# heliaxdev/ark-plonk

Hardware: AMD Instinct MI355X
Metric: proofs/sec at 2^20 constraints (BLS12-381, KZG10); MSM G1-adds/s (higher is better)
Workload: dtype u32 limbs (256/384-bit Montgomery integers)

## Files before the change

### ark_plonk_amd/csrc/fieldu.cuh

```cuda
#pragma once
#include "field_common.cuh"

template <class P>
struct Fu {
    static constexpr int NL = P::NL;
    static constexpr int SAT = P::SAT_WORDS;
    static constexpr uint32_t M = (1u << 29) - 1u;
    uint32_t v[NL];

    ZK_HD static Fu zero() {
        Fu r;
#pragma unroll
        for (int i = 0; i < NL; ++i) r.v[i] = 0;
        return r;
    }
    ZK_HD static Fu one() {
        Fu r;
#pragma unroll
        for (int i = 0; i < NL; ++i) r.v[i] = P::ONE(i);
        return r;
    }
    ZK_HD bool limbs_zero() const {
        uint32_t o = 0;
#pragma unroll
// ... 119 lines not shown
            t += (uint64_t)m[k] * P::MOD(0);
            carry = t >> 29;
        }
#pragma unroll
        for (int k = NL; k < 2 * NL - 1; ++k) {
            uint64_t a0 = 0, a1 = 0, am = 0;
#pragma unroll
            for (int i = k - NL + 1; i < NL; ++i) {
                if (i & 1) a1 += (uint64_t)a.v[i] * b.v[k - i];
                else a0 += (uint64_t)a.v[i] * b.v[k - i];
                am += (uint64_t)m[i] * P::MOD(k - i);
            }
            uint64_t t = a0 + a1 + am + carry;
            r.v[k - NL] = (uint32_t)t & M;
            carry = t >> 29;
        }
        r.v[NL - 1] = (uint32_t)carry;
        return r;
    }
    ZK_HD static uint64_t fence64(uint64_t t) {
#if defined(__HIP_DEVICE_COMPILE__)
        asm("" : "+v"(t));
#endif
        return t;
    }
    ZK_HD static Fu mul_fenced(const Fu& a, const Fu& b) {
        uint32_t m[NL];
        Fu r;
        uint64_t carry = 0;
#pragma unroll
        for (int k = 0; k < NL; ++k) {
            uint64_t t = fence64(carry + (uint64_t)a.v[0] * b.v[k]);
#pragma unroll
            for (int i = 1; i <= k; ++i) t += (uint64_t)a.v[i] * b.v[k - i];
#pragma unroll
            for (int i = 0; i < k; ++i) t += (uint64_t)m[i] * P::MOD(k - i);
            m[k] = ((uint32_t)t * P::PINV) & M;
            t += (uint64_t)m[k] * P::MOD(0);
            carry = t >> 29;
        }
#pragma unroll
        for (int k = NL; k < 2 * NL - 1; ++k) {
            uint64_t t = fence64(carry + (uint64_t)a.v[k - NL + 1] * b.v[NL - 1]);
#pragma unroll
            for (int i = k - NL + 2; i < NL; ++i) t += (uint64_t)a.v[i] * b.v[k - i];
#pragma unroll
            for (int i = k - NL + 1; i < NL; ++i) t += (uint64_t)m[i] * P::MOD(k - i);
            r.v[k - NL] = (uint32_t)t & M;
            carry = t >> 29;
        }
        r.v[NL - 1] = (uint32_t)carry;
        return r;
    }
    ZK_HD static Fu sqr(const Fu& a) {
        uint32_t m[NL], a2[NL];
        Fu r;
#pragma unroll
        for (int i = 0; i < NL; ++i) a2[i] = a.v[i] << 1;
        uint64_t carry = 0;
#pragma unroll
        for (int k = 0; k < NL; ++k) {
            uint64_t aa = 0, am = 0;
#pragma unroll
            for (int i = 0; 2 * i < k; ++i) aa += (uint64_t)a2[i] * a.v[k - i];
            if ((k & 1) == 0) aa += (uint64_t)a.v[k / 2] * a.v[k / 2];
#pragma unroll
            for (int i = 0; i < k; ++i) am += (uint64_t)m[i] * P::MOD(k - i);
            uint64_t t = aa + am + carry;
            m[k] = ((uint32_t)t * P::PINV) & M;
            t += (uint64_t)m[k] * P::MOD(0);
            carry = t >> 29;
        }
#pragma unroll
        for (int k = NL; k < 2 * NL - 1; ++k) {
            uint64_t aa = 0, am = 0;
#pragma unroll
            for (int i = k - NL + 1; 2 * i < k; ++i) aa += (uint64_t)a2[i] * a.v[k - i];
            if ((k & 1) == 0) aa += (uint64_t)a.v[k / 2] * a.v[k / 2];
#pragma unroll
            for (int i = k - NL + 1; i < NL; ++i) am += (uint64_t)m[i] * P::MOD(k - i);
            uint64_t t = aa + am + carry;
            r.v[k - NL] = (uint32_t)t & M;
            carry = t >> 29;
        }
        r.v[NL - 1] = (uint32_t)carry;
        return r;
    }

    ZK_HD bool is_zero_mod_reduced() const {
        if (v[0] != 0 && v[0] != P::MOD(0)) return false;
        uint32_t dz = 0, dp = 0;
#pragma unroll
        for (int i = 0; i < NL; ++i) {
            dz |= v[i];
            dp |= v[i] ^ P::MOD(i);
        }
        return dz == 0 || dp == 0;
    }
    ZK_HD bool is_zero_mod() const { return mul(*this, one()).is_zero_mod_reduced(); }

    ZK_HD static Fu canonical_lt2p(const Fu& a) {
        Fu d;
#pragma unroll
        for (int i = 0; i < NL; ++i) d.v[i] = a.v[i] - P::MOD(i);
        normalize(d);
        const bool neg = ((int32_t)d.v[NL - 1]) < 0;
// ... 46 lines not shown
```

### ark_plonk_amd/csrc/ntt.hip

```cpp
#include "ctx.h"
#include "domain.cuh"

#include "ntt_pass.cuh"

namespace {

template <class Fr>
struct PowBits {
    Fr p[32];
};
template <class Fr>
__global__ void gen_pow_table(void* out, uint64_t n, PowBits<Fr> pb, Fr mul, int mode, uint32_t log_m, uint32_t log_mprev, Fr to_rp) {
    uint64_t i = (uint64_t)blockIdx.x * blockDim.x + threadIdx.x;
    if (i >= n) return;
    uint64_t e = i;
    if (mode == 1) {
        uint64_t col = i & ((1ull << log_m) - 1);
        uint64_t k = i >> log_m;
        e = (col * k) & ((1ull << log_mprev) - 1);
    }
    Fr r = mul;
    for (int b = 0; b < 32; ++b) {
        if ((e >> b) & 1ull) r = Fr::mul(r, pb.p[b]);
    }
// ... 108 lines not shown
    if (hipMalloc(&p, cnt * TW_INNER_U4 * 16) != hipSuccess) {
        (void)hipFree(packed);
        return ZK_ERR_OOM;
    }
    Fr w = domain_root<C>((uint32_t)s);
    if (inverse) w = Fr::inverse(w);
    int rc = launch_pow_table<C>(c, packed, cnt, w, Fr::one(), 0, 0, 0);
    if (!rc) {
        const int T = 256;
        hipLaunchKernelGGL(split_table<typename C::FrU>, dim3((unsigned)((cnt + T - 1) / T)), dim3(T), 0, c->stream, packed, p, cnt);
        if (hipGetLastError() != hipSuccess || hipStreamSynchronize(c->stream) != hipSuccess) rc = ZK_ERR_HIP;
    }
    (void)hipFree(packed);
    if (rc) {
        (void)hipFree(p);
        return rc;
    }
    c->inner_tw[key] = p;
    *out = p;
    return ZK_OK;
}

template <class C>
int get_plan(zk_ctx* c, uint32_t log_n, bool inverse, NttPlan** out) {
    typedef typename C::Fr Fr;
    const int forced = forced_passes(c, log_n);
    uint64_t key = ((uint64_t)C::ID << 40) | ((uint64_t)forced << 36) | ((uint64_t)(inverse ? 1 : 0) << 32) | log_n;
    auto it = c->plans.find(key);
    if (it != c->plans.end()) {
        *out = it->second;
        return ZK_OK;
    }
    int n_pass, s[4];
    if (!decompose(log_n, forced, n_pass, s)) return ZK_ERR_UNSUPPORTED;
    NttPlan* pl = new NttPlan();
    pl->curve = C::ID;
    pl->log_n = log_n;
    pl->inverse = inverse;
    pl->n_pass = n_pass;
    for (int i = 0; i < 4; ++i) pl->s[i] = s[i];
    uint32_t log_mprev = log_n;
    for (int p = 0; p < pl->n_pass; ++p) {
        if (log_n >= 3) {
            int rc = get_inner_tw<C>(c, pl->s[p], inverse, &pl->tw_inner[p]);
            if (rc) { delete pl; return rc; }
        }
        if (p + 1 < pl->n_pass) {
            uint32_t log_m = log_mprev - (uint32_t)pl->s[p];
            uint64_t cnt = 1ull << log_mprev;
            hipError_t e = hipMalloc(&pl->tw_pass[p], cnt * sizeof(Fr));
            if (e != hipSuccess) { delete pl; return ZK_ERR_OOM; }
            Fr w = domain_root<C>(log_mprev);
            if (inverse) w = Fr::inverse(w);
            int rc = launch_pow_table<C>(c, pl->tw_pass[p], cnt, w, Fr::one(), 1, log_m, log_mprev);
            if (rc) { delete pl; return rc; }
            log_mprev = log_m;
        }
    }
    c->plans[key] = pl;
    *out = pl;
    return ZK_OK;
}

template <class C>
int ensure_coset(zk_ctx* c, bool inv, uint64_t len, void** out) {
    typedef typename C::Fr Fr;
    DevBuf& buf = inv ? c->coset_inv_pow[C::ID] : c->coset_pow[C::ID];
    size_t& have = inv ? c->coset_inv_len[C::ID] : c->coset_len[C::ID];
    if (have < len) {
        ZK_HIP_TRY(hipStreamSynchronize(c->stream));
        uint64_t want = 1;
        while (want < len) want <<= 1;
        int rc = buf.ensure(want * sizeof(Fr));
        if (rc) return rc;
        Fr g = coset_gen<C>();
        if (inv) g = Fr::inverse(g);
        rc = launch_pow_table<C>(c, buf.p, want, g, Fr::one(), 0, 0, 0);
        if (rc) return rc;
        have = want;
    }
    *out = buf.p;
    return ZK_OK;
}

typedef int (*NttPassLauncher)(int final_pass, const NttPassArgs* a, hipStream_t st);
extern "C" NttPassLauncher zk_ntt_pass_launcher(int curve, int s);

template <class C>
int dispatch_pass(zk_ctx* c, int s, bool final_pass, const NttPassArgs& a) {
    if (s < 3 || s > 9) return ZK_ERR_UNSUPPORTED;
    NttPassLauncher fn = zk_ntt_pass_launcher(C::ID, s);
    if (!fn) return ZK_ERR_UNSUPPORTED;
    hipError_t e = (hipError_t)fn(final_pass ? 1 : 0, &a, c->stream);
    ZK_HIP_TRY(e);
    return ZK_OK;
}

template <class C>
int ntt_run(zk_ctx* c, int kind, uint32_t log_n, uint32_t n_polys, const void* const* d_ins, const size_t* in_lens, void* const* d_outs) {
    typedef typename C::Fr Fr;
    if (!domain_log_ok<C>(log_n)) return ZK_ERR_DOMAIN_TOO_LARGE;
    if (n_polys == 0 || n_polys > 16) return ZK_ERR_BAD_ARG;
    const uint64_t N = 1ull << log_n;
    size_t in_len = 0;
    bool all_quarter = true;
    for (uint32_t i = 0; i < n_polys; ++i) {
        if (in_lens[i] > N) return ZK_ERR_BAD_ARG;
// ... 32 lines not shown
        rc = ensure_coset<C>(c, true, N, &post);
        if (rc) return rc;
    }
    NttPlan* pl = nullptr;
    rc = get_plan<C>(c, log_n, inverse, &pl);
    if (rc) return rc;
    if (pl->n_pass > 4) return ZK_ERR_UNSUPPORTED;
    void* work = nullptr;
    if (pl->n_pass > 1) {
        rc = c->ntt_work.ensure((size_t)n_polys * N * sizeof(Fr));
        if (rc) return rc;
        work = c->ntt_work.p;
    }
    uint32_t log_mprev = log_n;
    NttPassArgs a;
    ProfScope ps(c, "ntt_pass");
    for (int p = 0; p < pl->n_pass; ++p) {
        const int s = pl->s[p];
        const bool last = (p + 1 == pl->n_pass);
        memset(&a, 0, sizeof a);
        a.log_n = log_n;
        a.in = (p == 0) ? d_in : work;
        a.out = last ? d_out : work;
        a.in_len = (p == 0) ? in_lens[0] : N;
        if (n_polys > 1) {
            a.n_batch = n_polys;
            for (uint32_t i = 0; i < n_polys; ++i) {
                void* wk = (char*)work + (size_t)i * N * sizeof(Fr);
                a.ins[i] = (p == 0) ? d_ins[i] : wk;
                a.outs[i] = last ? d_outs[i] : wk;
                a.in_lens[i] = (p == 0) ? in_lens[i] : N;
            }
        }
        a.tw_inner = pl->tw_inner[p];
        a.pre_mul = (p == 0) ? pre : nullptr;
        const uint32_t LC = 9u - (uint32_t)s;
        if (!last) {
            uint32_t log_m = log_mprev - (uint32_t)s;
            uint32_t logc = LC < log_m ? LC : log_m;
            a.logc = logc;
            a.log_m = log_m;
            a.log_mprev = log_mprev;
            a.tw_pass = pl->tw_pass[p];
            a.n_tiles = (uint32_t)(N >> ((uint32_t)s + logc));
            a.quarter = (p == 0 && s >= 3 && all_quarter) ? 1u : 0u;
            log_mprev = log_m;
        } else {
            uint32_t s1 = (pl->n_pass > 1) ? (uint32_t)pl->s[0] : 0;
            uint32_t logc = LC < s1 ? LC : s1;
            a.logc = logc;
            a.s1 = s1;
            a.s2 = pl->n_pass == 4 ? (uint32_t)pl->s[1] : 0u;
            a.post_mul = post;
            const Fr sc = to_rprime(inverse ? n_inv : Fr::one());
            for (int i = 0; i < 8; ++i) a.scale[i] = sc.v[i];
            a.n_tiles = (uint32_t)(N >> ((uint32_t)s + logc));
        }
        rc = dispatch_pass<C>(c, s, last, a);
        if (rc) return rc;
        if (c->profiling) c->prof["ntt_passes"].launches += 1;
    }
    return ZK_OK;
}

}

int ntt_run_dev(zk_ctx* c, int curve, int kind, uint32_t log_n, const void* d_in, size_t in_len, void* d_out) {
    return ntt_run_batch_dev(c, curve, kind, log_n, 1, &d_in, &in_len, &d_out);
}

int ntt_run_batch_dev(zk_ctx* c, int curve, int kind, uint32_t log_n, uint32_t n_polys, const void* const* d_ins, const size_t* in_lens,
                      void* const* d_outs) {
    if (kind < 0 || kind > 3) return ZK_ERR_BAD_ARG;
    for (uint32_t base = 0; base < n_polys; base += 16) {
        const uint32_t cnt = n_polys - base < 16 ? n_polys - base : 16;
        const int rc = zk_on_curve(curve, ZK_ERR_BAD_ARG, [&](auto cv) {
            return ntt_run<decltype(cv)>(c, kind, log_n, cnt, d_ins + base, in_lens + base, d_outs + base);
        });
        if (rc) return rc;
    }
    return ZK_OK;
}

int ntt_prepare(zk_ctx* c, int curve, uint32_t log_n) {
    NttPlan* pl;
    if (log_n < 3) return ZK_OK;
    for (int inv = 0; inv < 2; ++inv) {
        const int rc = zk_on_curve(curve, ZK_ERR_BAD_ARG, [&](auto cv) {
            typedef decltype(cv) Cv;
            if (!domain_log_ok<Cv>(log_n)) return ZK_ERR_DOMAIN_TOO_LARGE;
            return get_plan<Cv>(c, log_n, inv != 0, &pl);
        });
        if (rc) return rc;
    }
    return ZK_OK;
}

void ntt_ctx_free(zk_ctx* c) {
    for (auto& kv : c->plans) delete kv.second;
    c->plans.clear();
    for (auto& kv : c->inner_tw) (void)hipFree(kv.second);
    c->inner_tw.clear();
    c->ntt_work.release();
    for (int i = 0; i < 2; ++i) {
        c->coset_pow[i].release();
        c->coset_inv_pow[i].release();
    }
}
// ... 34 lines not shown
```

### ark_plonk_amd/csrc/ntt_pass.cuh

```cuda
#pragma once
#include <hip/hip_runtime.h>
#include "curve_params.h"
#include "field.cuh"
#include "fieldu.cuh"

typedef __attribute__((address_space(3))) volatile uint32_t lds_u32;

struct NttPassArgs {
    const void* in;
    void* out;
    const void* tw_inner;
    const void* tw_pass;
    const void* pre_mul;
    const void* post_mul;
    uint32_t scale[8];
    uint64_t in_len;
    uint32_t log_n;
    uint32_t logc;
    uint32_t log_m;
    uint32_t log_mprev;
    uint32_t s1;
    uint32_t s2;
    uint32_t n_tiles;
    uint32_t quarter;
    uint32_t n_batch;
    const void* ins[16];
    void* outs[16];
    uint64_t in_lens[16];
};

__host__ __device__ inline uint32_t bitrev32(uint32_t x, int bits) {
#if defined(__HIP_DEVICE_COMPILE__)
    return bits ? __brev(x) >> (32 - bits) : 0u;
#else
    uint32_t r = 0;
    for (int i = 0; i < bits; ++i) { r = (r << 1) | (x & 1); x >>= 1; }
    return r;
#endif
}

template <class F>
ZK_D F ld_u(const void* base, uint64_t idx) {
    const uint4* q = reinterpret_cast<const uint4*>(base) + 2 * idx;
    uint4 a = q[0], b = q[1];
    uint32_t w[8] = {a.x, a.y, a.z, a.w, b.x, b.y, b.z, b.w};
    return F::split_words(w);
}
template <class F>
ZK_D void st_u(void* base, uint64_t idx, const F& x) {
    uint32_t w[8];
    F::canonical_lt2p(x).pack_words(w);
    uint4* q = reinterpret_cast<uint4*>(base) + 2 * idx;
    q[0] = make_uint4(w[0], w[1], w[2], w[3]);
    q[1] = make_uint4(w[4], w[5], w[6], w[7]);
}

template <class F>
ZK_D void st_u_raw(void* base, uint64_t idx, const F& x) {
    uint32_t w[8];
    x.pack_words(w);
    uint4* q = reinterpret_cast<uint4*>(base) + 2 * idx;
    q[0] = make_uint4(w[0], w[1], w[2], w[3]);
    q[1] = make_uint4(w[4], w[5], w[6], w[7]);
}

constexpr int TW_INNER_U4 = 3;
template <class F>
ZK_D F ld_limbs(const void* base, uint64_t idx) {
    static_assert(F::NL <= 4 * TW_INNER_U4, "inner twiddle entry too small");
    const uint4* q = reinterpret_cast<const uint4*>(base) + TW_INNER_U4 * idx;
    F r;
#pragma unroll
    for (int i = 0; i < TW_INNER_U4; ++i) {
        if (4 * i >= F::NL) break;
        const uint4 a = q[i];
        if (4 * i + 0 < F::NL) r.v[4 * i + 0] = a.x;
        if (4 * i + 1 < F::NL) r.v[4 * i + 1] = a.y;
// ... 19 lines not shown
ZK_D uint32_t window_pos(uint32_t v, uint32_t e) {
    return ((v >> B0) << (B0 + 3)) | (e << B0) | (v & ((1u << B0) - 1u));
}

template <class F>
ZK_D void wave_exchange(F (&x)[8], lds_u32* sc, const uint32_t (&widx)[8], const uint32_t (&ridx)[8]) {
#pragma unroll
    for (int l = 0; l < F::NL; ++l) {
#pragma unroll
        for (int e = 0; e < 8; ++e) sc[widx[e]] = x[e].v[l];
        __builtin_amdgcn_wave_barrier();
#pragma unroll
        for (int e = 0; e < 8; ++e) x[e].v[l] = sc[ridx[e]];
        __builtin_amdgcn_wave_barrier();
    }
}

template <class F, int S, int B0, int LB_LO, int LB_HI>
ZK_D void dit_window(F (&x)[8], uint32_t v, const void* tw, bool quarter) {
    const uint32_t vlow = v & ((1u << B0) - 1u);
#pragma unroll
    for (int lb = LB_LO; lb < LB_HI; ++lb) {
        const int t = B0 + lb;
        if (ntt_sweep_at(t)) {
#pragma unroll
            for (int e = 0; e < 8; ++e) F::sweep(x[e]);
        }
#pragma unroll
        for (int e = 0; e < 8; ++e) {
            if (e & (1 << lb)) continue;
            const int eo = e | (1 << lb);
            if constexpr (B0 == 0 && LB_LO == 0) {
                if (lb < 2 && quarter) {
                    x[eo] = x[e];
                    continue;
                }
                if (lb == 0) {
                    const F b = x[eo];
                    x[eo] = F::sub_raw3(x[e], b);
                    x[e] = F::add_raw(x[e], b);
                    continue;
                }
                if ((e & ((1 << lb) - 1)) == 0) {
                    F b = x[eo];
                    F::sweep(b);
                    x[eo] = lb == 1 ? F::sub_raw8(x[e], b) : F::sub_raw16(x[e], b);
                    x[e] = F::add_raw(x[e], b);
                    continue;
                }
            }
            const uint32_t plow = ((uint32_t)(e & ((1 << lb) - 1)) << B0) | vlow;
            const uint32_t j = plow << (S - 1 - t);
            F w = ld_limbs<F>(tw, j);
            F m = F::mul_fenced(x[eo], w);
            x[eo] = F::sub_raw3(x[e], m);
            x[e] = F::add_raw(x[e], m);
        }
    }
}

template <class F, int S, int B0>
ZK_D void dit_all(F (&x)[8], uint32_t v, uint32_t c, uint32_t LC, const void* tw, lds_u32* sc, bool quarter = false) {
    constexpr int REM = S - B0;
    if constexpr (REM >= 3) {
        dit_window<F, S, B0, 0, 3>(x, v, tw, quarter);
        if constexpr (REM > 3) {
            constexpr int NB0 = (REM - 3 >= 3) ? B0 + 3 : S - 3;
            uint32_t wi[8], ri[8];
#pragma unroll
            for (int e = 0; e < 8; ++e) {
                wi[e] = (window_pos<B0>(v, e) << LC) | c;
                ri[e] = (window_pos<NB0>(v, e) << LC) | c;
            }
            wave_exchange<F>(x, sc, wi, ri);
            if constexpr (REM - 3 >= 3) {
                dit_all<F, S, B0 + 3>(x, v, c, LC, tw, sc);
            } else {
                dit_window<F, S, S - 3, 3 - (REM - 3), 3>(x, v, tw, false);
            }
        }
    }
}

template <class F, int S>
__global__ void __launch_bounds__(256) ntt_pass_mid(NttPassArgs a) {
    constexpr uint32_t LC = 9 - S;
    __shared__ uint32_t scratch[4][512];
    const uint32_t lane = threadIdx.x & 63, wv = threadIdx.x >> 6;
    const uint32_t tile = blockIdx.x * (blockDim.x >> 6) + wv;
    if (tile >= a.n_tiles) return;
    const void* in = a.in;
    void* out = a.out;
    uint64_t in_len = a.in_len;
    if (a.n_batch) {
        in = a.ins[blockIdx.y];
        out = a.outs[blockIdx.y];
        in_len = a.in_lens[blockIdx.y];
    }
    lds_u32* sc = (lds_u32*)scratch[wv];
    const uint32_t c = lane & ((1u << LC) - 1u);
    const uint32_t v = lane >> LC;
    const bool active = c < (1u << a.logc);
    const uint32_t lcg = a.log_m - a.logc;
    const uint64_t blk = (uint64_t)tile >> lcg;
    const uint64_t cg = (uint64_t)tile & ((1ull << lcg) - 1);
    const uint64_t col = (cg << a.logc) + c;
    const uint64_t base = (blk << a.log_mprev) + col;

    F x[8];
#pragma unroll
    for (int e = 0; e < 8; ++e) {
        const uint64_t row = bitrev32((v << 3) | e, S);
        const uint64_t idx = base + (row << a.log_m);
        if (active && idx < in_len) {
            x[e] = ld_u<F>(in, idx);
            if (a.pre_mul) x[e] = F::mul_fenced(x[e], ld_u<F>(a.pre_mul, idx));
        } else {
            x[e] = F::zero();
        }
    }
    dit_all<F, S, 0>(x, v, c, LC, a.tw_inner, sc, a.quarter != 0);
    if (!active) return;
#pragma unroll
    for (int e = 0; e < 8; ++e) {
        const uint64_t k = S >= 3 ? (((uint64_t)e << (S - 3)) | v) : e;
        F w = ld_u<F>(a.tw_pass, (k << a.log_m) + col);
        if (ntt_units_before(S) > 6) F::sweep(x[e]);
        st_u_raw<F>(out, base + (k << a.log_m), F::mul_fenced(x[e], w));
    }
}

template <class F, int S>
__global__ void __launch_bounds__(256) ntt_pass_final(NttPassArgs a) {
    constexpr uint32_t L = 1u << S;
    constexpr uint32_t LC = 9 - S;
    __shared__ uint32_t scratch[4][512];
    const uint32_t lane = threadIdx.x & 63, wv = threadIdx.x >> 6;
    const uint32_t tile = blockIdx.x * (blockDim.x >> 6) + wv;
    if (tile >= a.n_tiles) return;
    const void* in = a.in;
    void* out = a.out;
    uint64_t in_len = a.in_len;
    if (a.n_batch) {
        in = a.ins[blockIdx.y];
        out = a.outs[blockIdx.y];
        in_len = a.in_lens[blockIdx.y];
    }
    lds_u32* sc = (lds_u32*)scratch[wv];
    const uint32_t log_nb = a.log_n - S;
    const uint32_t log_rest = log_nb - a.s1;
    const uint32_t lg = a.s1 - a.logc;
    const uint64_t rho = (uint64_t)tile >> lg;
    const uint64_t g = (uint64_t)tile & ((1ull << lg) - 1);

    F x[8];
    uint32_t wi[8], ri[8];
    const uint32_t c = lane & ((1u << LC) - 1u);
    const uint32_t v = lane >> LC;
#pragma unroll
    for (int e = 0; e < 8; ++e) {
        const uint32_t q = (uint32_t)e * 64u + lane;
        const uint32_t cb = q >> S, row = q & (L - 1);
        const uint64_t b = ((((uint64_t)g << a.logc) + cb) << log_rest) | rho;
        const uint64_t idx = (b << S) + row;
        if (cb < (1u << a.logc) && idx < in_len) {
            x[e] = ld_u<F>(in, idx);
            if (a.pre_mul) x[e] = F::mul_fenced(x[e], ld_u<F>(a.pre_mul, idx));
        } else {
            x[e] = F::zero();
        }
        wi[e] = (bitrev32(row, S) << LC) | cb;
        ri[e] = (((v << 3) | (uint32_t)e) << LC) | c;
    }
    wave_exchange<F>(x, sc, wi, ri);
    dit_all<F, S, 0>(x, v, c, LC, a.tw_inner, sc);
    if (c >= (1u << a.logc)) return;
    const uint64_t k1o = ((uint64_t)g << a.logc) + c;
    uint64_t rho_rev = rho;
    if (a.s2) {
        const uint32_t s3 = log_rest - a.s2;
        rho_rev = (rho >> s3) | ((rho & ((1ull << s3) - 1ull)) << a.s2);
    }
    const uint64_t obase = k1o + (rho_rev << a.s1);
    F sc_mul = F::split_words(a.scale);
#pragma unroll
    for (int e = 0; e < 8; ++e) {
        const uint64_t k = S >= 3 ? (((uint64_t)e << (S - 3)) | v) : e;
        const uint64_t oidx = obase + (k << log_nb);
        if (ntt_units_before(S) > 6) F::sweep(x[e]);
        F y = F::mul_fenced(x[e], sc_mul);
        if (a.post_mul) y = F::mul_fenced(y, ld_u<F>(a.post_mul, oidx));
        st_u<F>(out, oidx, y);
    }
}
```

### ark_plonk_amd/csrc/msm_sort.hip

```cpp
#include "msm_common.cuh"

namespace {

ZK_D uint32_t scalar_bits(const uint32_t (&s)[8], uint32_t pos, uint32_t c) {
    const uint32_t limb = pos >> 5, off = pos & 31;
    uint64_t lo = 0, hi = 0;
#pragma unroll
    for (int k = 0; k < 8; ++k) {
        if ((uint32_t)k == limb) lo = s[k];
        if ((uint32_t)k == limb + 1) hi = s[k];
    }
    const uint64_t v = ((hi << 32) | lo) >> off;
    return (uint32_t)v & ((1u << c) - 1u);
}

ZK_D bool scalar_fold(uint32_t (&k)[8], const MsmGeom& g) {
    if (!g.neg) return false;
#pragma unroll 1
    for (int it = 0; it < 6; ++it) {
        bool ge = true, dec = false;
#pragma unroll
        for (int i = 7; i >= 0; --i) {
            if (!dec && k[i] != g.mod[i]) {
                ge = k[i] > g.mod[i];
// ... 530 lines not shown
                sorted[q] = vr[k];
                skey[q] = (Lo)vk[k];
            }
        }
        __syncthreads();
#pragma unroll
        for (uint32_t k = 0; k < PER; ++k) {
            const uint32_t i = k * PS_T + t;
            if (i < m) {
                const uint32_t j = skey[i];
                entries[cur[j] + (i - toff[j])] = sorted[i];
            }
        }
        __syncthreads();
        for (uint32_t j = t; j < NB; j += PS_T) cur[j] += toff[j + 1] - toff[j];
    }
}


ZK_D uint32_t cs_bits(const uint32_t (&s)[8], uint32_t w) {
    const uint32_t pos = w * CS_C, limb = pos >> 5, off = pos & 31;
    uint64_t v = s[limb < 8 ? limb : 7];
    if (limb >= 8) v = 0;
    if (limb + 1 < 8) v |= (uint64_t)s[limb + 1] << 32;
    return (uint32_t)(v >> off) & ((1u << CS_C) - 1u);
}

template <class Fr, bool MONT>
__global__ void __launch_bounds__(256, 8) csort_fold_hist(const uint32_t* scalars, uint64_t n, uint32_t sp, MsmGeom g, uint4* folded,
                                                       uint32_t* hist , uint32_t* scan_counter, uint32_t* combine_q) {
    __shared__ uint32_t lc[PS_PARTS];
    reset_job_counters(scan_counter, combine_q);
    lc[threadIdx.x] = 0;
    __syncthreads();
    const uint64_t lo = slab_lo(n, sp), hi = slab_hi(lo, n, sp);
    for (uint64_t i = lo + threadIdx.x; i < hi; i += 256) {
        Fr x = ld_scalar<Fr, MONT>(scalars, i);
        const bool flip = scalar_fold(x.v, g);
        uint32_t carry = 0;
#pragma unroll
        for (uint32_t w = 0; w < 16; ++w) {
            if (w < g.W) {
                const uint32_t mag = recode(cs_bits(x.v, w), carry, CS_C).mag;
                if (mag != 0) atomicAdd(&lc[(mag - 1) >> CS_LOB], 1u);
            }
        }
        folded[2 * i] = make_uint4(x.v[0], x.v[1], x.v[2], x.v[3]);
        folded[2 * i + 1] = make_uint4(x.v[4], x.v[5], x.v[6], x.v[7] | (flip ? 0x80000000u : 0u));
    }
    __syncthreads();
    hist[(uint64_t)threadIdx.x * PS_SLABS + blockIdx.x] = lc[threadIdx.x];
}

__global__ void __launch_bounds__(PS_T, 8) csort_scatter(SJobs jobs, uint32_t W) {
    extern __shared__ uint32_t rec[];
    const SJob& J = jobs.j[blockIdx.y];
    const uint4* folded = (const uint4*)J.dig;
    const uint64_t n = J.n;
    const uint32_t sp = J.sp;
    const uint32_t* cursors = J.hist;
    const uint32_t* part_start = J.part_start;
    uint32_t* stage = J.stage_ref;
    constexpr uint32_t LOM = (1u << CS_LOB) - 1u;
    __shared__ uint32_t cnt[PS_PARTS], toff[PS_PARTS + 1], gcur[PS_PARTS], stmp[4];
    const uint32_t t = threadIdx.x;
    if (t < 256) gcur[t] = part_start[t] + cursors[(uint64_t)t * PS_SLABS + blockIdx.x];
    const uint64_t lo = slab_lo(n, sp), hi = slab_hi(lo, n, sp);
    const uint32_t len = (uint32_t)(hi - lo);
    uint4 na = make_uint4(0, 0, 0, 0), nb = na;
    auto fetch = [&](uint32_t tb) {
        if (tb + t < len) {
            na = folded[2 * (lo + tb + t)];
            nb = folded[2 * (lo + tb + t) + 1];
        }
    };
    if (len) fetch(0);
    for (uint32_t tb = 0; tb < len; tb += PS_T) {
        __syncthreads();
        if (t < 256) cnt[t] = 0;
        __syncthreads();
        const bool have = tb + t < len;
        uint32_t s[8] = {na.x, na.y, na.z, na.w, nb.x, nb.y, nb.z, nb.w & 0x7fffffffu};
        const uint32_t flip = nb.w >> 31;
        if (tb + PS_T < len) fetch(tb + PS_T);
        uint32_t pk[16];
        uint32_t carry = 0;
#pragma unroll
        for (uint32_t w = 0; w < 16; ++w) {
            pk[w] = 0xffffffffu;
            if (have && w < W) {
                const Digit d = recode(cs_bits(s, w), carry, CS_C, flip);
                if (d.mag != 0) {
                    const uint32_t b = d.mag - 1;
                    pk[w] = ((b >> CS_LOB) << 23) | (d.neg << 22) | (w << 18) | (t << 8) | (b & LOM);
                    atomicAdd(&cnt[b >> CS_LOB], 1u);
                }
            }
        }
        tile_offsets256(cnt, toff, stmp, t);
#pragma unroll
        for (uint32_t w = 0; w < 16; ++w)
            if (pk[w] != 0xffffffffu) rec[atomicAdd(&cnt[pk[w] >> 23], 1u)] = pk[w];
        __syncthreads();
        const uint32_t total = toff[256];
#pragma unroll
        for (uint32_t k = 0; k < 16; ++k) {
            const uint32_t qq = k * PS_T + t;
            if (qq < total) {
                const uint32_t r = rec[qq];
                const uint32_t pp = r >> 23;
                const uint32_t rel = tb + ((r >> 8) & (PS_T - 1u));
                stage[gcur[pp] + (qq - toff[pp])] = cs_pack((r >> 22) & 1u, (r >> 18) & 15u, rel, r & LOM);
            }
        }
        __syncthreads();
        advance_cursors256(gcur, toff, t);
    }
}

constexpr uint32_t CS_RT = 4;
__global__ void __launch_bounds__(PS_T) csort_final(SJobs jobs) {
    extern __shared__ uint32_t lds[];
    const SJob& J = jobs.j[blockIdx.y];
    const uint32_t* stage = J.stage_ref;
    const uint32_t* part_start = J.part_start;
    uint32_t* entries = J.entries;
    uint32_t* offsets = J.offsets;
    const uint32_t n = (uint32_t)J.n, sp = J.sp;
    constexpr uint32_t PER = PS_TILE / PS_T, NB = 1u << CS_LOB, LOM = NB - 1u;
    static_assert(NB == 256 && PS_SLABS == 1024 && PS_T == PS_SLABS && CS_RT * NB == PS_T, "one slab cursor and one (tile, bucket) per lane");
    __shared__ uint32_t pos[CS_RT * NB];
    __shared__ uint32_t dst[CS_RT * NB];
    __shared__ uint32_t tmp_a[16], tmp_b[16];
    uint32_t* curs = lds;
    uint32_t* sorted = curs + PS_SLABS + 1;
    uint8_t* skey = reinterpret_cast<uint8_t*>(sorted + PS_TILE);
    uint16_t* slab_of = reinterpret_cast<uint16_t*>(skey + PS_TILE);
    const uint32_t p = blockIdx.x, t = threadIdx.x;
    const uint32_t s = part_start[p], e = part_start[p + 1];
    const uint32_t len = e - s;
    if (len > CS_RT * PS_TILE) return;
    uint32_t all[CS_RT][PER];
    {
        const uint32_t* mine = stage + s + t;
#pragma unroll
        for (uint32_t r = 0; r < CS_RT; ++r)
#pragma unroll
            for (uint32_t k = 0; k < PER; ++k) {
                const uint32_t i = (r * PER + k) * PS_T;
                if (i + t < len) all[r][k] = mine[i];
            }
    }
    curs[t] = J.hist[(uint64_t)p * PS_SLABS + t];
    if (t == 0) curs[PS_SLABS] = len;
    pos[t] = 0;
    __syncthreads();
#pragma unroll
    for (uint32_t r = 0; r < CS_RT; ++r)
#pragma unroll
        for (uint32_t k = 0; k < PER; ++k)
            if ((r * PER + k) * PS_T + t < len) atomicAdd(&pos[r * NB + (all[r][k] & LOM)], 1u);
    __syncthreads();
    {
        const uint32_t r = t >> 8, j = t & (NB - 1u), wv = t >> 6;
        const uint32_t c = pos[t];
        uint32_t before = 0, total = 0;
#pragma unroll
        for (uint32_t q = 0; q < CS_RT; ++q) {
            const uint32_t v = pos[q * NB + j];
            if (q < r) before += v;
            total += v;
        }
        uint32_t inc_a = c, inc_b = total;
#pragma unroll
        for (uint32_t d = 1; d < 64; d <<= 1) {
            const uint32_t oa = __shfl_up(inc_a, d, 64), ob = __shfl_up(inc_b, d, 64);
            if ((t & 63) >= d) {
                inc_a += oa;
                inc_b += ob;
            }
        }
        if ((t & 63) == 63) {
            tmp_a[wv] = inc_a;
            tmp_b[wv] = inc_b;
        }
        __syncthreads();
        uint32_t add_a = 0, add_b = 0;
        for (uint32_t w = wv & ~3u; w < wv; ++w) {
            add_a += tmp_a[w];
            add_b += tmp_b[w];
        }
        const uint32_t in_tile = inc_a + add_a - c;
        const uint32_t start = s + inc_b + add_b - total;
        pos[t] = in_tile;
        dst[t] = start + before - in_tile;
        if (r == 0) offsets[p * NB + j] = start;
        if (p == PS_PARTS - 1 && t == 0) offsets[PS_PARTS * NB] = e;
    }
    const uint32_t run0 = curs[t], run1 = curs[t + 1];
    auto mark_slabs = [&](uint32_t a0) {
        const uint32_t a1 = a0 + PS_TILE < len ? a0 + PS_TILE : len, l = t & 63;
        const uint32_t r0 = run0 > a0 ? run0 : a0, r1 = run1 < a1 ? run1 : a1;
        const bool wide = r1 > r0 && r1 - r0 > 64;
        if (!wide)
            for (uint32_t q = r0; q < r1; ++q) slab_of[q - a0] = (uint16_t)t;
        unsigned long long todo = __ballot(wide);
        while (todo) {
            const int src = __ffsll((long long)todo) - 1;
            todo &= todo - 1;
            const uint32_t b0 = __shfl(r0, src, 64), b1 = __shfl(r1, src, 64);
            for (uint32_t q = b0 + l; q < b1; q += 64) slab_of[q - a0] = (uint16_t)((t & ~63u) + (uint32_t)src);
        }
    };
    mark_slabs(0);
    __syncthreads();
#pragma unroll
    for (uint32_t r = 0; r < CS_RT; ++r) {
        if (r * PS_TILE >= len) break;
        const uint32_t m = len - r * PS_TILE < PS_TILE ? len - r * PS_TILE : PS_TILE;
#pragma unroll
        for (uint32_t k = 0; k < PER; ++k) {
            const uint32_t i = k * PS_T + t;
            if (i < m) {
                const uint32_t v = all[r][k];
                const uint32_t slab = slab_of[i];
                const uint32_t q = atomicAdd(&pos[r * NB + (v & LOM)], 1u);
                sorted[q] = cs_ref(v, slab, sp, n);
                skey[q] = (uint8_t)(v & LOM);
            }
        }
        __syncthreads();
#pragma unroll
        for (uint32_t k = 0; k < PER; ++k) {
            const uint32_t i = k * PS_T + t;
            if (i < m) entries[dst[r * NB + skey[i]] + i] = sorted[i];
        }
        if ((r + 1) * PS_TILE < len) mark_slabs((r + 1) * PS_TILE);
        __syncthreads();
    }
}

__global__ void __launch_bounds__(PS_T) csort_final_long(SJobs jobs) {
    extern __shared__ uint32_t lds[];
    const SJob& J = jobs.j[blockIdx.y];
    const uint32_t* stage = J.stage_ref;
    const uint32_t* part_start = J.part_start;
    uint32_t* entries = J.entries;
    uint32_t* offsets = J.offsets;
    const uint32_t n = (uint32_t)J.n, sp = J.sp;
    constexpr uint32_t PER = PS_TILE / PS_T, NB = 1u << CS_LOB, LOM = NB - 1u;
    static_assert(NB == 256 && PS_SLABS == 1024 && PS_T == PS_SLABS, "tile_offsets256; one slab cursor per lane; 10-step search");
    __shared__ uint32_t cnt[NB], cur[NB], toff[NB + 1], stmp[4];
    uint32_t* curs = lds;
    uint32_t* sorted = curs + PS_SLABS;
    uint8_t* skey = reinterpret_cast<uint8_t*>(sorted + PS_TILE);
    const uint32_t p = blockIdx.x, t = threadIdx.x;
    const uint32_t s = part_start[p], e = part_start[p + 1];
    if (e - s <= CS_RT * PS_TILE) return;
    curs[t] = J.hist[(uint64_t)p * PS_SLABS + t];
    if (t < NB) cnt[t] = 0;
    __syncthreads();
    count_keys(stage, s + t, e, cnt, LOM);
    __syncthreads();
    {
        const uint32_t ex = scan256_excl(t < NB ? cnt[t] : 0u, t, stmp);
        if (t < NB) cur[t] = s + ex;
    }
    __syncthreads();
    if (t < NB) offsets[p * NB + t] = cur[t];
    if (p == PS_PARTS - 1 && t == 0) offsets[PS_PARTS * NB] = e;
    uint32_t nr[PER];
    auto fetch = [&](uint32_t base) {
        const uint32_t m = e - base < PS_TILE ? e - base : PS_TILE;
#pragma unroll
        for (uint32_t k = 0; k < PER; ++k) {
            const uint32_t i = k * PS_T + t;
            if (i < m) nr[k] = stage[base + i];
        }
    };
    if (s < e) fetch(s);
    for (uint32_t base = s; base < e; base += PS_TILE) {
        const uint32_t m = e - base < PS_TILE ? e - base : PS_TILE;
        __syncthreads();
        if (t < NB) cnt[t] = 0;
        __syncthreads();
        uint32_t vr[PER];
#pragma unroll
        for (uint32_t k = 0; k < PER; ++k) vr[k] = nr[k];
        if (base + PS_TILE < e) fetch(base + PS_TILE);
#pragma unroll
        for (uint32_t k = 0; k < PER; ++k) {
// ... 92 lines not shown
                               pk.combine_q);
        else
            hipLaunchKernelGGL((psort_digits_hist<FrS, MONT, int16_t>), grid, block, 0, st, scalars, (uint64_t)n, sp, pl.g, lob, (int16_t*)dig, hist,
                               pk.scan_counter, pk.combine_q);
    });
    ZK_HIP_TRY(hipGetLastError());
    return ZK_OK;
}

template <class Dig, class Lo, uint32_t LOB>
int queue_psort_passes(const SJobs& sj, uint32_t n_jobs, const MsmGeom& g, hipStream_t st) {
    const uint32_t lob = g.c - 9;
    const size_t lds = LOB ? 0 : psort_final_lds(lob, sizeof(Lo));
    hipLaunchKernelGGL((psort_scatter<Dig, Lo, LOB>), dim3(PS_SLABS, n_jobs), dim3(PS_T), 0, st, sj, g.W, lob);
    if (lds) ZK_HIP_TRY(hipFuncSetAttribute((const void*)psort_final<Lo, LOB>, hipFuncAttributeMaxDynamicSharedMemorySize, (int)lds));
    hipLaunchKernelGGL((psort_final<Lo, LOB>), dim3(PS_PARTS, n_jobs), dim3(PS_T), lds, st, sj, lob);
    return ZK_OK;
}

template <class Cv>
int pre_queue_sort_rest(zk_ctx* c, const PrePlan* pls, MsmBufs* const* mbs, const size_t* lens, uint32_t n_jobs, hipStream_t st) {
    if (n_jobs == 0) return ZK_OK;
    if (n_jobs > (uint32_t)MAX_JOBS) return ZK_ERR_UNSUPPORTED;
    uint32_t n_shared = 0;
    for (uint32_t k = 0; k < n_jobs; ++k) n_shared += pls[k].shared_stage ? 1u : 0u;
    if (n_shared && n_jobs > 1) {
        for (uint32_t k = 0; k < n_jobs; ++k) {
            int rc = pre_queue_sort_rest<Cv>(c, pls + k, mbs + k, lens + k, 1, st);
            if (rc) return rc;
        }
        return ZK_OK;
    }
    ProfScope ps(c, "msm_sort", st);
    const PrePlan& p0 = pls[0];
    SJobs sj;
    memset(&sj, 0, sizeof sj);
    for (uint32_t k = 0; k < n_jobs; ++k) {
        MsmBufs& mb = *mbs[k];
        SJob& J = sj.j[k];
        const PartKey pk(mb);
        void* stage = pls[k].shared_stage ? c->stage_shared.p : mb.stage.p;
        J.dig = mb.entries.p;
        J.n = lens[k];
        J.sp = psort_slab_len(lens[k]);
        J.hist = (uint32_t*)mb.counts.p;
        J.part_start = pk.part_start;
        J.part_total = pk.part_total;
        J.counter = pk.scan_counter;
        J.stage_ref = (uint32_t*)stage;
        J.stage_lo = (char*)stage + (size_t)pls[k].nf * 4;
        J.entries = (uint32_t*)mb.entries.p;
        J.offsets = (uint32_t*)mb.offsets.p;
    }
    hipLaunchKernelGGL(psort_scan, dim3(PS_PARTS, n_jobs), dim3(PS_SLABS), 0, st, sj);
    if (pre_compact(p0)) {
        const size_t lds_s = (size_t)p0.g.W * PS_T * 4, lds_f = ((size_t)PS_SLABS + 1 + PS_TILE) * 4 + (size_t)PS_TILE * 3,
                     lds_l = ((size_t)PS_SLABS + PS_TILE) * 4 + PS_TILE;
        ZK_HIP_TRY(hipFuncSetAttribute((const void*)csort_scatter, hipFuncAttributeMaxDynamicSharedMemorySize, (int)lds_s));
        hipLaunchKernelGGL(csort_scatter, dim3(PS_SLABS, n_jobs), dim3(PS_T), lds_s, st, sj, p0.g.W);
        ZK_HIP_TRY(hipFuncSetAttribute((const void*)csort_final, hipFuncAttributeMaxDynamicSharedMemorySize, (int)lds_f));
        hipLaunchKernelGGL(csort_final, dim3(PS_PARTS, n_jobs), dim3(PS_T), lds_f, st, sj);
        ZK_HIP_TRY(hipFuncSetAttribute((const void*)csort_final_long, hipFuncAttributeMaxDynamicSharedMemorySize, (int)lds_l));
        hipLaunchKernelGGL(csort_final_long, dim3(PS_PARTS, n_jobs), dim3(PS_T), lds_l, st, sj);
    } else {
        const int rc = p0.wide ? queue_psort_passes<int32_t, uint16_t, 0>(sj, n_jobs, p0.g, st)
                               : queue_psort_passes<int16_t, uint8_t, PRE_C - 9>(sj, n_jobs, p0.g, st);
        if (rc) return rc;
    }
    ZK_HIP_TRY(hipGetLastError());
    return ZK_OK;
}

}

int ZK_SYM(pw_queue_sort)(zk_ctx* c, const MsmGeom& g, uint32_t S, MsmBufs& mb, const void* d_scalars, size_t n, hipStream_t st) {
    return pw_queue_sort<CurveSel>(c, g, S, mb, d_scalars, n, st);
}
int ZK_SYM(pre_queue_digits)(zk_ctx* c, const PrePlan& pl, MsmBufs& mb, const void* d_scalars, size_t n, hipStream_t st, bool mont) {
    return pre_queue_digits<CurveSel>(c, pl, mb, d_scalars, n, st, mont);
}
int ZK_SYM(pre_queue_sort_rest)(zk_ctx* c, const PrePlan* pls, MsmBufs* const* mbs, const size_t* lens, uint32_t n_jobs, hipStream_t st) {
    return pre_queue_sort_rest<CurveSel>(c, pls, mbs, lens, n_jobs, st);
}
```

Baseline: 13.26.

## Fold inverse NTT scale into twiddles and replace final-pass multiply with cheap reduction

The inverse-NTT 1/n scale is folded into the last inter-pass twiddle table, or applied on input when there is only one pass. The final pass no longer multiplies every output by a scale constant and instead reduces lazily accumulated values with a cheap quotient-estimate reduction (reduce_47p). Field multiplications in the NTT passes switch from the fenced Montgomery multiply to a new chained-accumulation variant that uses empty asm to force serial accumulation. This removes one full Montgomery multiply per output element but relies on the reduce_47p bound (values below 47p) and the changed twiddle generation being correct.

```diff
diff --git a/ark_plonk_amd/csrc/fieldu.cuh b/ark_plonk_amd/csrc/fieldu.cuh
--- a/ark_plonk_amd/csrc/fieldu.cuh
+++ b/ark_plonk_amd/csrc/fieldu.cuh
@@ -195,6 +195,59 @@
         r.v[NL - 1] = (uint32_t)carry;
         return r;
     }
+    ZK_HD static uint64_t link(uint64_t t) {
+#if defined(__HIP_DEVICE_COMPILE__)
+        asm volatile("" : : "v"(t));
+#endif
+        return t;
+    }
+    ZK_HD static Fu mul_chain(const Fu& a, const Fu& b) {
+        uint32_t m[NL];
+        Fu r;
+        uint64_t carry = 0;
+#pragma unroll
+        for (int k = 0; k < NL; ++k) {
+            uint64_t t = (uint64_t)a.v[0] * b.v[k];
+            if (k) t = link(carry + t);
+#pragma unroll
+            for (int i = 1; i <= k; ++i) t = link(t + (uint64_t)a.v[i] * b.v[k - i]);
+#pragma unroll
+            for (int i = 0; i < k; ++i) t = link(t + (uint64_t)m[i] * P::MOD(k - i));
+            m[k] = ((uint32_t)t * P::PINV) & M;
+            t += (uint64_t)m[k] * P::MOD(0);
+            carry = t >> 29;
+        }
+#pragma unroll
+        for (int k = NL; k < 2 * NL - 1; ++k) {
+            uint64_t t = link(carry + (uint64_t)a.v[k - NL + 1] * b.v[NL - 1]);
+#pragma unroll
+            for (int i = k - NL + 2; i < NL; ++i) t = link(t + (uint64_t)a.v[i] * b.v[k - i]);
+#pragma unroll
+            for (int i = k - NL + 1; i < NL; ++i) t = link(t + (uint64_t)m[i] * P::MOD(k - i));
+            r.v[k - NL] = (uint32_t)t & M;
+            carry = t >> 29;
+        }
+        r.v[NL - 1] = (uint32_t)carry;
+        return r;
+    }
+
+    static constexpr uint32_t TOP1 = P::MOD(NL - 1) + 1;
+    static constexpr uint32_t QMAGIC = (uint32_t)((1ull << 52) / TOP1) + 1u;
+    static_assert(47ull * TOP1 * TOP1 <= (1ull << 52) && (1ull << 52) / TOP1 < 0xffffffffull && P::MOD(NL - 1) >= 47, "quot_top's constant");
+    ZK_HD static uint32_t quot_top(uint32_t x_top) { return (uint32_t)(((uint64_t)x_top * QMAGIC) >> 52); }
+    ZK_HD static constexpr uint32_t NEG_MOD(int i) { return i == 0 ? (1u << 29) - P::MOD(0) : M - P::MOD(i); }
+    ZK_HD static Fu reduce_47p(const Fu& x) {
+        const uint32_t q = quot_top(x.v[NL - 1]);
+        Fu y;
+        uint32_t c = 0;
+#pragma unroll
+        for (int i = 0; i < NL; ++i) {
+            const uint64_t t = (uint64_t)q * NEG_MOD(i) + (x.v[i] + c);
+            y.v[i] = (uint32_t)t & M;
+            c = (uint32_t)(t >> 29);
+        }
+        return y;
+    }
     ZK_HD static Fu sqr(const Fu& a) {
         uint32_t m[NL], a2[NL];
         Fu r;
diff --git a/ark_plonk_amd/csrc/ntt.hip b/ark_plonk_amd/csrc/ntt.hip
--- a/ark_plonk_amd/csrc/ntt.hip
+++ b/ark_plonk_amd/csrc/ntt.hip
@@ -184,7 +184,8 @@
             if (e != hipSuccess) { delete pl; return ZK_ERR_OOM; }
             Fr w = domain_root<C>(log_mprev);
             if (inverse) w = Fr::inverse(w);
-            int rc = launch_pow_table<C>(c, pl->tw_pass[p], cnt, w, Fr::one(), 1, log_m, log_mprev);
+            const Fr mul = (inverse && p + 2 == pl->n_pass) ? Fr::inverse(Fr::from_u64(1ull << log_n)) : Fr::one();
+            int rc = launch_pow_table<C>(c, pl->tw_pass[p], cnt, w, mul, 1, log_m, log_mprev);
             if (rc) { delete pl; return rc; }
             log_mprev = log_m;
         }
@@ -323,8 +324,11 @@
             a.s1 = s1;
             a.s2 = pl->n_pass == 4 ? (uint32_t)pl->s[1] : 0u;
             a.post_mul = post;
-            const Fr sc = to_rprime(inverse ? n_inv : Fr::one());
-            for (int i = 0; i < 8; ++i) a.scale[i] = sc.v[i];
+            if (inverse && pl->n_pass == 1) {
+                const Fr sc = to_rprime(n_inv);
+                for (int i = 0; i < 8; ++i) a.scale[i] = sc.v[i];
+                a.scale_in = 1;
+            }
             a.n_tiles = (uint32_t)(N >> ((uint32_t)s + logc));
         }
         rc = dispatch_pass<C>(c, s, last, a);
diff --git a/ark_plonk_amd/csrc/ntt_pass.cuh b/ark_plonk_amd/csrc/ntt_pass.cuh
--- a/ark_plonk_amd/csrc/ntt_pass.cuh
+++ b/ark_plonk_amd/csrc/ntt_pass.cuh
@@ -23,6 +23,7 @@
     uint32_t s2;
     uint32_t n_tiles;
     uint32_t quarter;
+    uint32_t scale_in;
     uint32_t n_batch;
     const void* ins[16];
     void* outs[16];
@@ -148,7 +149,7 @@
             const uint32_t plow = ((uint32_t)(e & ((1 << lb) - 1)) << B0) | vlow;
             const uint32_t j = plow << (S - 1 - t);
             F w = ld_limbs<F>(tw, j);
-            F m = F::mul_fenced(x[eo], w);
+            F m = F::mul_chain(x[eo], w);
             x[eo] = F::sub_raw3(x[e], m);
             x[e] = F::add_raw(x[e], m);
         }
@@ -210,7 +211,7 @@
         const uint64_t idx = base + (row << a.log_m);
         if (active && idx < in_len) {
             x[e] = ld_u<F>(in, idx);
-            if (a.pre_mul) x[e] = F::mul_fenced(x[e], ld_u<F>(a.pre_mul, idx));
+            if (a.pre_mul) x[e] = F::mul_chain(x[e], ld_u<F>(a.pre_mul, idx));
         } else {
             x[e] = F::zero();
         }
@@ -222,7 +223,7 @@
         const uint64_t k = S >= 3 ? (((uint64_t)e << (S - 3)) | v) : e;
         F w = ld_u<F>(a.tw_pass, (k << a.log_m) + col);
         if (ntt_units_before(S) > 6) F::sweep(x[e]);
-        st_u_raw<F>(out, base + (k << a.log_m), F::mul_fenced(x[e], w));
+        st_u_raw<F>(out, base + (k << a.log_m), F::mul_chain(x[e], w));
     }
 }
 
@@ -249,6 +250,7 @@
     const uint64_t rho = (uint64_t)tile >> lg;
     const uint64_t g = (uint64_t)tile & ((1ull << lg) - 1);
 
+    const F sc_mul = F::split_words(a.scale);
     F x[8];
     uint32_t wi[8], ri[8];
     const uint32_t c = lane & ((1u << LC) - 1u);
@@ -261,7 +263,7 @@
         const uint64_t idx = (b << S) + row;
         if (cb < (1u << a.logc) && idx < in_len) {
             x[e] = ld_u<F>(in, idx);
-            if (a.pre_mul) x[e] = F::mul_fenced(x[e], ld_u<F>(a.pre_mul, idx));
+            if (a.pre_mul || a.scale_in) x[e] = F::mul_chain(x[e], a.pre_mul ? ld_u<F>(a.pre_mul, idx) : sc_mul);
         } else {
             x[e] = F::zero();
         }
@@ -278,14 +280,18 @@
         rho_rev = (rho >> s3) | ((rho & ((1ull << s3) - 1ull)) << a.s2);
     }
     const uint64_t obase = k1o + (rho_rev << a.s1);
-    F sc_mul = F::split_words(a.scale);
 #pragma unroll
     for (int e = 0; e < 8; ++e) {
         const uint64_t k = S >= 3 ? (((uint64_t)e << (S - 3)) | v) : e;
         const uint64_t oidx = obase + (k << log_nb);
-        if (ntt_units_before(S) > 6) F::sweep(x[e]);
-        F y = F::mul_fenced(x[e], sc_mul);
-        if (a.post_mul) y = F::mul_fenced(y, ld_u<F>(a.post_mul, oidx));
+        F y;
+        if (a.post_mul) {
+            if (ntt_units_before(S) > 6) F::sweep(x[e]);
+            y = F::mul_chain(x[e], ld_u<F>(a.post_mul, oidx));
+        } else {
+            F::sweep(x[e]);
+            y = F::reduce_47p(x[e]);
+        }
         st_u<F>(out, oidx, y);
     }
 }
```

After: 13.34, median of 6. No clear change (+0.6%).

## Split compact-sort scan and loop csort_final over jobs with prefetch

Applied to the files above, without the earlier changes.

In the compact path, the general psort_scan is replaced by a lighter csort_scan that scans each partition's slab counts with vectorized uint4 loads. The cross-partition prefix of part_start is moved into csort_scatter, whose block 0 also writes it out. csort_final now launches one block per partition and loops over all jobs, loading the next job's stage tile into registers while the current job is being processed. This is meant to cut scan cost and hide global load latency, at the price of less grid parallelism and more register pressure.

```diff
diff --git a/ark_plonk_amd/csrc/msm_sort.hip b/ark_plonk_amd/csrc/msm_sort.hip
--- a/ark_plonk_amd/csrc/msm_sort.hip
+++ b/ark_plonk_amd/csrc/msm_sort.hip
@@ -606,6 +606,19 @@
     hist[(uint64_t)threadIdx.x * PS_SLABS + blockIdx.x] = lc[threadIdx.x];
 }
 
+constexpr uint32_t CSCAN_T = PS_SLABS / 4;
+__global__ void __launch_bounds__(CSCAN_T) csort_scan(SJobs jobs) {
+    static_assert(CSCAN_T == 256, "scan256_excl over the lanes' sums");
+    __shared__ uint32_t tmp[4];
+    const uint32_t t = threadIdx.x;
+    uint4* row = reinterpret_cast<uint4*>(jobs.j[blockIdx.y].hist + (uint64_t)blockIdx.x * PS_SLABS);
+    const uint4 v = row[t];
+    const uint32_t sum = v.x + v.y + v.z + v.w;
+    const uint32_t ex = scan256_excl(sum, t, tmp);
+    row[t] = make_uint4(ex, ex + v.x, ex + v.x + v.y, ex + v.x + v.y + v.z);
+    if (t == CSCAN_T - 1) jobs.j[blockIdx.y].part_total[blockIdx.x] = ex + sum;
+}
+
 __global__ void __launch_bounds__(PS_T, 8) csort_scatter(SJobs jobs, uint32_t W) {
     extern __shared__ uint32_t rec[];
     const SJob& J = jobs.j[blockIdx.y];
@@ -613,12 +626,22 @@
     const uint64_t n = J.n;
     const uint32_t sp = J.sp;
     const uint32_t* cursors = J.hist;
-    const uint32_t* part_start = J.part_start;
+    uint32_t* part_start = J.part_start;
     uint32_t* stage = J.stage_ref;
     constexpr uint32_t LOM = (1u << CS_LOB) - 1u;
     __shared__ uint32_t cnt[PS_PARTS], toff[PS_PARTS + 1], gcur[PS_PARTS], stmp[4];
     const uint32_t t = threadIdx.x;
-    if (t < 256) gcur[t] = part_start[t] + cursors[(uint64_t)t * PS_SLABS + blockIdx.x];
+    {
+        const uint32_t total = t < 256 ? J.part_total[t] : 0u;
+        const uint32_t start = scan256_excl(total, t, stmp);
+        if (t < 256) {
+            gcur[t] = start + cursors[(uint64_t)t * PS_SLABS + blockIdx.x];
+            if (blockIdx.x == 0) {
+                part_start[t] = start;
+                if (t == 255) part_start[PS_PARTS] = start + total;
+            }
+        }
+    }
     const uint64_t lo = slab_lo(n, sp), hi = slab_hi(lo, n, sp);
     const uint32_t len = (uint32_t)(hi - lo);
     uint4 na = make_uint4(0, 0, 0, 0), nb = na;
@@ -673,14 +696,8 @@
 }
 
 constexpr uint32_t CS_RT = 4;
-__global__ void __launch_bounds__(PS_T) csort_final(SJobs jobs) {
+__global__ void __launch_bounds__(PS_T) csort_final(SJobs jobs, uint32_t n_jobs) {
     extern __shared__ uint32_t lds[];
-    const SJob& J = jobs.j[blockIdx.y];
-    const uint32_t* stage = J.stage_ref;
-    const uint32_t* part_start = J.part_start;
-    uint32_t* entries = J.entries;
-    uint32_t* offsets = J.offsets;
-    const uint32_t n = (uint32_t)J.n, sp = J.sp;
     constexpr uint32_t PER = PS_TILE / PS_T, NB = 1u << CS_LOB, LOM = NB - 1u;
     static_assert(NB == 256 && PS_SLABS == 1024 && PS_T == PS_SLABS && CS_RT * NB == PS_T, "one slab cursor and one (tile, bucket) per lane");
     __shared__ uint32_t pos[CS_RT * NB];
@@ -690,107 +707,135 @@
     uint32_t* sorted = curs + PS_SLABS + 1;
     uint8_t* skey = reinterpret_cast<uint8_t*>(sorted + PS_TILE);
     uint16_t* slab_of = reinterpret_cast<uint16_t*>(skey + PS_TILE);
-    const uint32_t p = blockIdx.x, t = threadIdx.x;
-    const uint32_t s = part_start[p], e = part_start[p + 1];
-    const uint32_t len = e - s;
-    if (len > CS_RT * PS_TILE) return;
+    const uint32_t p = blockIdx.x, lane = threadIdx.x;
+    uint32_t ns = 0, nlen = 0, ncur = 0;
+    bool nlong = false;
+    const uint32_t* nmine = nullptr;
+    auto open_job = [&](uint32_t y) {
+        nlen = 0;
+        nlong = false;
+        if (y >= n_jobs) return;
+        const SJob& N = jobs.j[y];
+        ns = N.part_start[p];
+        const uint32_t l = N.part_start[p + 1] - ns;
+        nlong = l > CS_RT * PS_TILE;
+        if (nlong) return;
+        nlen = l;
+        ncur = N.hist[(uint64_t)p * PS_SLABS + lane];
+        nmine = N.stage_ref + ns + lane;
+    };
     uint32_t all[CS_RT][PER];
-    {
-        const uint32_t* mine = stage + s + t;
+    auto load_tile = [&](uint32_t (&a)[PER], uint32_t r) {
+#pragma unroll
+        for (uint32_t k = 0; k < PER; ++k) {
+            const uint32_t i = (r * PER + k) * PS_T;
+            if (i + lane < nlen) a[k] = nmine[i];
+        }
+    };
+    open_job(0);
+#pragma unroll
+    for (uint32_t r = 0; r < CS_RT; ++r) load_tile(all[r], r);
+#pragma unroll 1
+    for (uint32_t y = 0; y < n_jobs; ++y) {
+        uint32_t t = lane;
+        asm volatile("" : "+v"(t));
+        const SJob& J = jobs.j[y];
+        uint32_t* entries = J.entries;
+        uint32_t* offsets = J.offsets;
+        const uint32_t n = (uint32_t)J.n, sp = J.sp;
+        const uint32_t s = ns, len = nlen, e = s + len;
+        const bool is_long = nlong;
+        const uint32_t cur0 = ncur;
+        open_job(y + 1);
+        curs[t] = cur0;
+        if (t == 0) curs[PS_SLABS] = len;
+        pos[t] = 0;
+        __syncthreads();
 #pragma unroll
         for (uint32_t r = 0; r < CS_RT; ++r)
 #pragma unroll
-            for (uint32_t k = 0; k < PER; ++k) {
-                const uint32_t i = (r * PER + k) * PS_T;
-                if (i + t < len) all[r][k] = mine[i];
-            }
-    }
-    curs[t] = J.hist[(uint64_t)p * PS_SLABS + t];
-    if (t == 0) curs[PS_SLABS] = len;
-    pos[t] = 0;
-    __syncthreads();
-#pragma unroll
-    for (uint32_t r = 0; r < CS_RT; ++r)
-#pragma unroll
-        for (uint32_t k = 0; k < PER; ++k)
-            if ((r * PER + k) * PS_T + t < len) atomicAdd(&pos[r * NB + (all[r][k] & LOM)], 1u);
-    __syncthreads();
-    {
-        const uint32_t r = t >> 8, j = t & (NB - 1u), wv = t >> 6;
-        const uint32_t c = pos[t];
-        uint32_t before = 0, total = 0;
-#pragma unroll
-        for (uint32_t q = 0; q < CS_RT; ++q) {
-            const uint32_t v = pos[q * NB + j];
-            if (q < r) before += v;
-            total += v;
-        }
-        uint32_t inc_a = c, inc_b = total;
-#pragma unroll
-        for (uint32_t d = 1; d < 64; d <<= 1) {
-            const uint32_t oa = __shfl_up(inc_a, d, 64), ob = __shfl_up(inc_b, d, 64);
-            if ((t & 63) >= d) {
-                inc_a += oa;
-                inc_b += ob;
-            }
-        }
-        if ((t & 63) == 63) {
-            tmp_a[wv] = inc_a;
-            tmp_b[wv] = inc_b;
-        }
-        __syncthreads();
-        uint32_t add_a = 0, add_b = 0;
-        for (uint32_t w = wv & ~3u; w < wv; ++w) {
-            add_a += tmp_a[w];
-            add_b += tmp_b[w];
-        }
-        const uint32_t in_tile = inc_a + add_a - c;
-        const uint32_t start = s + inc_b + add_b - total;
-        pos[t] = in_tile;
-        dst[t] = start + before - in_tile;
-        if (r == 0) offsets[p * NB + j] = start;
-        if (p == PS_PARTS - 1 && t == 0) offsets[PS_PARTS * NB] = e;
-    }
-    const uint32_t run0 = curs[t], run1 = curs[t + 1];
-    auto mark_slabs = [&](uint32_t a0) {
-        const uint32_t a1 = a0 + PS_TILE < len ? a0 + PS_TILE : len, l = t & 63;
-        const uint32_t r0 = run0 > a0 ? run0 : a0, r1 = run1 < a1 ? run1 : a1;
-        const bool wide = r1 > r0 && r1 - r0 > 64;
-        if (!wide)
-            for (uint32_t q = r0; q < r1; ++q) slab_of[q - a0] = (uint16_t)t;
-        unsigned long long todo = __ballot(wide);
-        while (todo) {
-            const int src = __ffsll((long long)todo) - 1;
-            todo &= todo - 1;
-            const uint32_t b0 = __shfl(r0, src, 64), b1 = __shfl(r1, src, 64);
-            for (uint32_t q = b0 + l; q < b1; q += 64) slab_of[q - a0] = (uint16_t)((t & ~63u) + (uint32_t)src);
-        }
-    };
-    mark_slabs(0);
-    __syncthreads();
-#pragma unroll
-    for (uint32_t r = 0; r < CS_RT; ++r) {
-        if (r * PS_TILE >= len) break;
-        const uint32_t m = len - r * PS_TILE < PS_TILE ? len - r * PS_TILE : PS_TILE;
-#pragma unroll
-        for (uint32_t k = 0; k < PER; ++k) {
-            const uint32_t i = k * PS_T + t;
-            if (i < m) {
-                const uint32_t v = all[r][k];
-                const uint32_t slab = slab_of[i];
-                const uint32_t q = atomicAdd(&pos[r * NB + (v & LOM)], 1u);
-                sorted[q] = cs_ref(v, slab, sp, n);
-                skey[q] = (uint8_t)(v & LOM);
-            }
-        }
-        __syncthreads();
-#pragma unroll
-        for (uint32_t k = 0; k < PER; ++k) {
-            const uint32_t i = k * PS_T + t;
-            if (i < m) entries[dst[r * NB + skey[i]] + i] = sorted[i];
-        }
-        if ((r + 1) * PS_TILE < len) mark_slabs((r + 1) * PS_TILE);
-        __syncthreads();
+            for (uint32_t k = 0; k < PER; ++k)
+                if ((r * PER + k) * PS_T + t < len) atomicAdd(&pos[r * NB + (all[r][k] & LOM)], 1u);
+        __syncthreads();
+        {
+            const uint32_t r = t >> 8, j = t & (NB - 1u), wv = t >> 6;
+            const uint32_t c = pos[t];
+            uint32_t before = 0, total = 0;
+#pragma unroll
+            for (uint32_t q = 0; q < CS_RT; ++q) {
+                const uint32_t v = pos[q * NB + j];
+                if (q < r) before += v;
+                total += v;
+            }
+            uint32_t inc_a = c, inc_b = total;
+#pragma unroll
+            for (uint32_t d = 1; d < 64; d <<= 1) {
+                const uint32_t oa = __shfl_up(inc_a, d, 64), ob = __shfl_up(inc_b, d, 64);
+                if ((t & 63) >= d) {
+                    inc_a += oa;
+                    inc_b += ob;
+                }
+            }
+            if ((t & 63) == 63) {
+                tmp_a[wv] = inc_a;
+                tmp_b[wv] = inc_b;
+            }
+            __syncthreads();
+            uint32_t add_a = 0, add_b = 0;
+            for (uint32_t w = wv & ~3u; w < wv; ++w) {
+                add_a += tmp_a[w];
+                add_b += tmp_b[w];
+            }
+            const uint32_t in_tile = inc_a + add_a - c;
+            const uint32_t start = s + inc_b + add_b - total;
+            pos[t] = in_tile;
+            dst[t] = start + before - in_tile;
+            if (r == 0 && !is_long) offsets[p * NB + j] = start;
+            if (p == PS_PARTS - 1 && t == 0 && !is_long) offsets[PS_PARTS * NB] = e;
+        }
+        const uint32_t run0 = curs[t], run1 = curs[t + 1];
+        auto mark_slabs = [&](uint32_t a0) {
+            const uint32_t a1 = a0 + PS_TILE < len ? a0 + PS_TILE : len, l = t & 63;
+            const uint32_t r0 = run0 > a0 ? run0 : a0, r1 = run1 < a1 ? run1 : a1;
+            const bool wide = r1 > r0 && r1 - r0 > 64;
+            if (!wide)
+                for (uint32_t q = r0; q < r1; ++q) slab_of[q - a0] = (uint16_t)t;
+            unsigned long long todo = __ballot(wide);
+            while (todo) {
+                const int src = __ffsll((long long)todo) - 1;
+                todo &= todo - 1;
+                const uint32_t b0 = __shfl(r0, src, 64), b1 = __shfl(r1, src, 64);
+                for (uint32_t q = b0 + l; q < b1; q += 64) slab_of[q - a0] = (uint16_t)((t & ~63u) + (uint32_t)src);
+            }
+        };
+        mark_slabs(0);
+        __syncthreads();
+#pragma unroll
+        for (uint32_t r = 0; r < CS_RT; ++r) {
+            if (r * PS_TILE < len) {
+                const uint32_t m = len - r * PS_TILE < PS_TILE ? len - r * PS_TILE : PS_TILE;
+#pragma unroll
+                for (uint32_t k = 0; k < PER; ++k) {
+                    const uint32_t i = k * PS_T + t;
+                    if (i < m) {
+                        const uint32_t v = all[r][k];
+                        const uint32_t slab = slab_of[i];
+                        const uint32_t q = atomicAdd(&pos[r * NB + (v & LOM)], 1u);
+                        sorted[q] = cs_ref(v, slab, sp, n);
+                        skey[q] = (uint8_t)(v & LOM);
+                    }
+                }
+                __syncthreads();
+#pragma unroll
+                for (uint32_t k = 0; k < PER; ++k) {
+                    const uint32_t i = k * PS_T + t;
+                    if (i < m) entries[dst[r * NB + skey[i]] + i] = sorted[i];
+                }
+                if ((r + 1) * PS_TILE < len) mark_slabs((r + 1) * PS_TILE);
+                __syncthreads();
+            }
+            load_tile(all[r], r);
+        }
     }
 }
 
@@ -989,17 +1034,18 @@
         J.entries = (uint32_t*)mb.entries.p;
         J.offsets = (uint32_t*)mb.offsets.p;
     }
-    hipLaunchKernelGGL(psort_scan, dim3(PS_PARTS, n_jobs), dim3(PS_SLABS), 0, st, sj);
     if (pre_compact(p0)) {
+        hipLaunchKernelGGL(csort_scan, dim3(PS_PARTS, n_jobs), dim3(CSCAN_T), 0, st, sj);
         const size_t lds_s = (size_t)p0.g.W * PS_T * 4, lds_f = ((size_t)PS_SLABS + 1 + PS_TILE) * 4 + (size_t)PS_TILE * 3,
                      lds_l = ((size_t)PS_SLABS + PS_TILE) * 4 + PS_TILE;
         ZK_HIP_TRY(hipFuncSetAttribute((const void*)csort_scatter, hipFuncAttributeMaxDynamicSharedMemorySize, (int)lds_s));
         hipLaunchKernelGGL(csort_scatter, dim3(PS_SLABS, n_jobs), dim3(PS_T), lds_s, st, sj, p0.g.W);
         ZK_HIP_TRY(hipFuncSetAttribute((const void*)csort_final, hipFuncAttributeMaxDynamicSharedMemorySize, (int)lds_f));
-        hipLaunchKernelGGL(csort_final, dim3(PS_PARTS, n_jobs), dim3(PS_T), lds_f, st, sj);
+        hipLaunchKernelGGL(csort_final, dim3(PS_PARTS), dim3(PS_T), lds_f, st, sj, n_jobs);
         ZK_HIP_TRY(hipFuncSetAttribute((const void*)csort_final_long, hipFuncAttributeMaxDynamicSharedMemorySize, (int)lds_l));
         hipLaunchKernelGGL(csort_final_long, dim3(PS_PARTS, n_jobs), dim3(PS_T), lds_l, st, sj);
     } else {
+        hipLaunchKernelGGL(psort_scan, dim3(PS_PARTS, n_jobs), dim3(PS_SLABS), 0, st, sj);
         const int rc = p0.wide ? queue_psort_passes<int32_t, uint16_t, 0>(sj, n_jobs, p0.g, st)
                                : queue_psort_passes<int16_t, uint8_t, PRE_C - 9>(sj, n_jobs, p0.g, st);
         if (rc) return rc;
```

Result: no change. 12.83 before, 12.87 after (median of 3 runs) (+0.3%).
